# hanmekim/SceneLib2

Hardware: AMD Instinct MI355X
Metric: batched MonoSLAM frames/sec (320x240, 100 feat) (higher is better)
Workload: dtype f64

## Files before the change

### include/scenelib2_amd_testing.h

```cpp
#ifndef SCENELIB2_AMD_TESTING_H
#define SCENELIB2_AMD_TESTING_H
#include "scenelib2_amd.h"
#ifdef __cplusplus
extern "C" {
#endif

int sl2_set_feature_counters(sl2_engine* e, int seq, int label, int attempted, int successful);

int sl2_debug_set_position_error(sl2_engine* e, int seq, int label, int err);

int sl2_debug_graph_captures(sl2_engine* e);

int sl2_debug_update_plan(sl2_engine* e, int group, int* out, int n);

int sl2_debug_raw_covariance(sl2_engine* e, int seq, double* P, int capacity_ld, int* ld);

int sl2_debug_ncc_score(int device, const int32_t* sums5, int count, double* score, double* sd0, double* sd1);
int sl2_debug_gemm_kt(int device, const double* XT, int ldx, const double* YT, int ldy, int M, int N, int K,
                      double* C, int ldc);

int sl2_debug_microbench(int device, int which, double* result);

#define SL2_FRAME_MONITOR_BAND_ROWS 32

#ifdef __cplusplus
}
#endif
#endif
```

### scenelib2_amd/_lib.py

```python
import ctypes as C
import os

import numpy as np

_HERE = os.path.dirname(os.path.abspath(__file__))
LIB_PATH = os.environ.get("SL2_LIB_PATH") or os.path.join(_HERE, "libscenelib2_amd.so")

SL2_OK = 0
SL2_ERR_INVALID = 1
SL2_ERR_HIP = 2
SL2_ERR_CAPACITY = 3
SL2_ERR_NO_DEVICE = 4


class Sl2Error(RuntimeError):
    def __init__(self, code, msg):
        super().__init__("scenelib2_amd error %d: %s" % (code, msg))
        self.code = code


class sl2_camera(C.Structure):
    _fields_ = [("width", C.c_int32), ("height", C.c_int32), ("fku", C.c_double), ("fkv", C.c_double),
                ("u0", C.c_double), ("v0", C.c_double), ("kd1", C.c_double), ("sd", C.c_int32)]

# ... 106 lines not shown
                               ("rgb", np.uint8, (3,)), ("pad", np.uint8), ("q", np.float64, (4,))])
assert OVERLAY_ITEM_DTYPE.itemsize == 64
SL2_WORLD_TRAJECTORY, SL2_WORLD_FEATURES, SL2_WORLD_UNCERTAINTIES, SL2_WORLD_CAMERA, SL2_WORLD_AXES, SL2_WORLD_ALL = 1, 2, 4, 8, 16, 31


class sl2_view(C.Structure):
    _fields_ = [("r", C.c_double * 3), ("q", C.c_double * 4), ("fku", C.c_double), ("fkv", C.c_double), ("u0", C.c_double),
                ("v0", C.c_double)]


VIEW_DTYPE = np.dtype([("r", np.float64, (3,)), ("q", np.float64, (4,)), ("fku", np.float64), ("fkv", np.float64),
                       ("u0", np.float64), ("v0", np.float64)])
assert C.sizeof(sl2_view) == 88 and VIEW_DTYPE.itemsize == 88

SL2_BLOB_MAGIC = 0x51324C53
SL2_BLOB_SLOT_ARRAYS = 22
SL2_BLOB_LAYOUT_OFFSETS = 7 + SL2_BLOB_SLOT_ARRAYS

assert C.sizeof(sl2_snapshot_header) == 256 and C.sizeof(sl2_partial_info) == 32 and C.sizeof(sl2_sequence_blob_header) == 256
assert C.sizeof(sl2_step_stats) == 96 and STEP_STATS_DTYPE.itemsize == 96
assert C.sizeof(sl2_frame_source) == 24

EXPORTED_SYMBOLS = [
    "sl2_api_version", "sl2_device_count", "sl2_create", "sl2_destroy", "sl2_last_error", "sl2_synchronize", "sl2_batch",
    "sl2_max_features", "sl2_set_vehicle_state", "sl2_get_vehicle_state", "sl2_add_known_features", "sl2_set_feature_covariances",
    "sl2_go_one_step", "sl2_initialise_feature", "sl2_initialise_auto_feature", "sl2_save_patch", "sl2_set_groups", "sl2_set_search_variant", "sl2_set_step_fusion", "sl2_get_stream", "sl2_set_search_split", "sl2_set_update_variant", "sl2_set_graph_mode", "sl2_kalman_filter_predict", "sl2_auto_select_n_features", "sl2_make_measurements",
    "sl2_kalman_filter_update", "sl2_finish_step", "sl2_elliptical_search_batch", "sl2_find_best_patch_batch",
    "sl2_search_multiple_overlapping_ellipses_batch", "sl2_list_frames", "sl2_read_pgm", "sl2_read_image", "sl2_ingest_open",
    "sl2_ingest_frame_count", "sl2_ingest_next", "sl2_ingest_set_zero_copy", "sl2_ingest_close", "sl2_get_total_state_sizes",
    "sl2_get_total_state", "sl2_get_total_covariance", "sl2_get_features", "sl2_get_partial_feature", "sl2_get_selection",
    "sl2_snapshot_capacity", "sl2_snapshot", "sl2_get_trajectory", "sl2_get_feature_patch", "sl2_get_position_log", "sl2_delete_features", "sl2_get_status_flags", "sl2_set_profiling", "sl2_set_profile_focus",
    "sl2_reset_kernel_times", "sl2_kernel_count", "sl2_get_kernel_time", "sl2_get_step_work", "sl2_get_placement",
    "sl2_synth_render_host", "sl2_synth_render_device", "sl2_dev_malloc", "sl2_dev_free", "sl2_dev_upload",
    "sl2_dev_download",
    "sl2_sequence_blob_layout", "sl2_sequence_blob_capacity", "sl2_save_sequences", "sl2_load_sequences", "sl2_copy_sequences",
    "sl2_reset_sequences",
    "sl2_set_active_sequences", "sl2_get_active_sequences", "sl2_ingest_frame_counts", "sl2_ingest_next_ragged",
    "sl2_get_step_stats",
    "sl2_set_delta_t", "sl2_get_delta_t", "sl2_set_pause_catch_up",
    "sl2_set_cameras", "sl2_get_cameras",
    "sl2_converter_create", "sl2_converter_destroy", "sl2_converter_set_sources", "sl2_converter_get_sources",
    "sl2_convert_frames", "sl2_convert_frame_host", "sl2_scale_camera",
    "sl2_converter_set_filters", "sl2_converter_get_filters", "sl2_convert_frame_host_filtered",
    "sl2_snapshot_bound", "sl2_snapshot_batch",
    "sl2_overlay_item_bound", "sl2_overlay_items", "sl2_draw_items_batch", "sl2_draw_overlays", "sl2_draw_items_host",
    "sl2_rectify_frames", "sl2_rectify_frame_host", "sl2_scene_item_bound", "sl2_scene_items", "sl2_draw_rectified",
    "sl2_view_look_at", "sl2_world_item_bound", "sl2_world_items", "sl2_draw_world", "sl2_pick_items_batch", "sl2_pick_items_host",
    "sl2_converter_set_map", "sl2_converter_set_remaps", "sl2_converter_get_remaps", "sl2_remap_frame_host",
    "sl2_lens_map_host", "sl2_lens_pinhole_camera",
    "sl2_frame_monitor_create", "sl2_frame_monitor_destroy", "sl2_frame_monitor_set_gates", "sl2_frame_monitor_get_gates",
    "sl2_frame_monitor_reset", "sl2_examine_frames", "sl2_frame_monitor_read", "sl2_frame_stats_host", "sl2_frame_verdict_host",
]
TEST_SYMBOLS = ["sl2_set_feature_counters", "sl2_debug_set_position_error", "sl2_debug_ncc_score", "sl2_debug_gemm_kt", "sl2_debug_microbench", "sl2_debug_graph_captures",
                "sl2_debug_update_plan", "sl2_debug_raw_covariance"]
TEST_LIB_PATH = os.path.join(_HERE, "libscenelib2_amd_test.so")
_testlib = None

_lib = None

c_dp = C.POINTER(C.c_double)
c_ip = C.POINTER(C.c_int32)
c_u8p = C.POINTER(C.c_uint8)
vp = C.c_void_p


def dp(a):
    return a.ctypes.data_as(c_dp)


def ip(a):
    return a.ctypes.data_as(c_ip)


def u8p(a):
    return a.ctypes.data_as(c_u8p)


def _bind(L):
    L.sl2_last_error.restype = C.c_char_p
    L.sl2_device_count.restype = C.c_int
    L.sl2_create.argtypes = [C.POINTER(sl2_camera), C.POINTER(sl2_params), C.c_int, C.c_int, C.c_int, vp, C.POINTER(vp)]
    L.sl2_destroy.argtypes = [vp]
    L.sl2_destroy.restype = None
    L.sl2_synchronize.argtypes = [vp]
    L.sl2_batch.argtypes = [vp]
    L.sl2_max_features.argtypes = [vp]
    L.sl2_set_vehicle_state.argtypes = [vp, C.c_int, C.c_int, c_dp, c_dp]
    L.sl2_get_vehicle_state.argtypes = [vp, C.c_int, C.c_int, c_dp, c_dp]
    L.sl2_add_known_features.argtypes = [vp, C.c_int, C.c_int, C.c_int, c_dp, c_dp, c_u8p]
    L.sl2_set_feature_covariances.argtypes = [vp, C.c_int, C.c_int, C.c_int, c_dp]
    L.sl2_go_one_step.argtypes = [vp, vp, C.c_size_t, C.c_int, C.c_int, C.c_int]
    L.sl2_set_groups.argtypes = [vp, C.c_int]
    L.sl2_set_search_variant.argtypes = [vp, C.c_int]
    if "SL2_LIB_PATH" not in os.environ or hasattr(L, "sl2_set_search_split"):
        L.sl2_set_search_split.argtypes = [vp, C.c_int]
    L.sl2_set_update_variant.argtypes = [vp, C.c_int, C.c_int]
    L.sl2_set_graph_mode.argtypes = [vp, C.c_int]
    L.sl2_set_step_fusion.argtypes = [vp, C.c_int]
    L.sl2_get_stream.argtypes = [vp]
    L.sl2_get_stream.restype = vp
    L.sl2_kalman_filter_predict.argtypes = [vp]
    L.sl2_auto_select_n_features.argtypes = [vp, C.c_int]
    L.sl2_make_measurements.argtypes = [vp, vp, C.c_size_t, C.c_int]
    L.sl2_kalman_filter_update.argtypes = [vp]
    L.sl2_finish_step.argtypes = [vp, C.c_int]
    L.sl2_elliptical_search_batch.argtypes = [C.c_int, c_u8p, C.c_int, C.c_int, C.c_int, c_ip, c_u8p, c_dp, c_dp,
                                              C.c_int, c_ip, c_ip, c_dp, C.c_int]
# ... 92 lines not shown
        L.sl2_overlay_item_bound.argtypes = [C.c_int, C.c_int]
        L.sl2_overlay_item_bound.restype = C.c_size_t
        L.sl2_overlay_items.argtypes = [vp, C.c_int, C.c_int, C.c_int, vp, vp, C.c_int, vp, C.c_int]
        L.sl2_draw_items_batch.argtypes = [C.c_int, vp, vp, C.c_int, C.c_int, C.c_int, C.c_int, C.c_size_t, vp, C.c_int, vp, C.c_int,
                                           vp, C.c_size_t, C.c_int, vp, C.c_size_t, C.c_int]
        L.sl2_draw_overlays.argtypes = [vp, C.c_int, C.c_int, vp, C.c_size_t, C.c_int, C.c_int, vp, vp, C.c_size_t, C.c_int]
        L.sl2_draw_items_host.argtypes = [vp, C.c_int, C.c_int, vp, C.c_int, vp, C.c_size_t, C.c_int, vp]
    if "SL2_LIB_PATH" not in os.environ or hasattr(L, "sl2_rectify_frames"):
        L.sl2_rectify_frames.argtypes = [vp, C.c_int, C.c_int, vp, C.c_size_t, C.c_int, vp, C.c_size_t, C.c_int]
        L.sl2_rectify_frame_host.argtypes = [vp, C.c_int, C.c_int, C.c_double, C.c_double, C.c_double, vp]
        L.sl2_scene_item_bound.argtypes = [C.c_int, C.c_int]
        L.sl2_scene_item_bound.restype = C.c_size_t
        L.sl2_scene_items.argtypes = [vp, C.c_int, C.c_int, C.c_int, vp, vp, C.c_int, vp, C.c_int]
        L.sl2_draw_rectified.argtypes = [vp, C.c_int, C.c_int, vp, C.c_size_t, C.c_int, C.c_int, vp, vp, C.c_size_t, C.c_int]
    if "SL2_LIB_PATH" not in os.environ or hasattr(L, "sl2_world_items"):
        L.sl2_view_look_at.argtypes = [c_dp, c_dp, c_dp, C.c_double, C.c_double, C.c_double, C.c_double, vp]
        L.sl2_world_item_bound.argtypes = [C.c_int, C.c_int]
        L.sl2_world_item_bound.restype = C.c_size_t
        L.sl2_world_items.argtypes = [vp, C.c_int, C.c_int, vp, C.c_int, C.c_int, vp, vp, C.c_int, vp, vp, C.c_int]
        L.sl2_draw_world.argtypes = [vp, C.c_int, C.c_int, vp, C.c_int, C.c_int, C.c_int, C.c_int, C.c_int, vp, vp, C.c_size_t, C.c_int]
        L.sl2_pick_items_batch.argtypes = [C.c_int, vp, C.c_int, C.c_int, C.c_int, vp, C.c_int, vp, C.c_int, vp, vp, C.c_int]
        L.sl2_pick_items_host.argtypes = [C.c_int, C.c_int, vp, C.c_int, C.c_int, C.c_int, C.c_int, vp]
    if "SL2_LIB_PATH" not in os.environ or hasattr(L, "sl2_examine_frames"):
        L.sl2_frame_monitor_create.argtypes = [C.c_int, C.c_int, C.c_int, C.c_int, C.POINTER(vp)]
        L.sl2_frame_monitor_destroy.argtypes = [vp]
        L.sl2_frame_monitor_destroy.restype = None
        L.sl2_frame_monitor_set_gates.argtypes = [vp, C.c_int, C.c_int, C.POINTER(sl2_frame_gate)]
        L.sl2_frame_monitor_get_gates.argtypes = [vp, C.c_int, C.c_int, C.POINTER(sl2_frame_gate)]
        L.sl2_frame_monitor_reset.argtypes = [vp, C.c_int, C.c_int]
        L.sl2_examine_frames.argtypes = [vp, vp, vp, C.c_size_t, vp, vp, vp, vp]
        L.sl2_frame_monitor_read.argtypes = [vp, C.c_int, C.c_int, vp, vp]
        L.sl2_frame_stats_host.argtypes = [vp, C.c_int, C.c_int, C.POINTER(sl2_frame_stats)]
        L.sl2_frame_verdict_host.argtypes = [C.POINTER(sl2_frame_stats), C.POINTER(sl2_frame_gate), C.c_int, C.c_uint64]
        L.sl2_frame_verdict_host.restype = C.c_uint32
    return L


def load_testing():
    global _testlib
    if _testlib is not None:
        return _testlib
    load()
    if not os.path.exists(TEST_LIB_PATH):
        raise ImportError("scenelib2_amd: %s not built (make -C scenelib2_amd/csrc)" % TEST_LIB_PATH)
    T = _bind(C.CDLL(TEST_LIB_PATH))
    T.sl2_set_feature_counters.argtypes = [vp, C.c_int, C.c_int, C.c_int, C.c_int]
    T.sl2_debug_set_position_error.argtypes = [vp, C.c_int, C.c_int, C.c_int]
    T.sl2_debug_ncc_score.argtypes = [C.c_int, c_ip, C.c_int, c_dp, c_dp, c_dp]
    T.sl2_debug_gemm_kt.argtypes = [C.c_int, c_dp, C.c_int, c_dp, C.c_int, C.c_int, C.c_int, C.c_int, c_dp, C.c_int]
    T.sl2_debug_microbench.argtypes = [C.c_int, C.c_int, c_dp]
    T.sl2_debug_graph_captures.argtypes = [vp]
    T.sl2_debug_update_plan.argtypes = [vp, C.c_int, c_ip, C.c_int]
    T.sl2_debug_raw_covariance.argtypes = [vp, C.c_int, c_dp, C.c_int, c_ip]
    _testlib = T
    return T


def load():
    global _lib
    if _lib is not None:
        return _lib
    if not os.path.exists(LIB_PATH):
        raise ImportError("scenelib2_amd: native library %s not built (run __graft_entry__.build() or "
                          "`make -C scenelib2_amd/csrc`); there is no CPU fallback" % LIB_PATH)
    _lib = _bind(C.CDLL(LIB_PATH))
    return _lib


def check(rc, L=None):
    if rc != SL2_OK:
        raise Sl2Error(rc, (L or load()).sl2_last_error().decode("utf-8", "replace"))


def device_count():
    return load().sl2_device_count()


def make_camera(cam):
    return sl2_camera(int(cam["width"]), int(cam["height"]), float(cam["fku"]), float(cam["fkv"]),
                      float(cam["u0"]), float(cam["v0"]), float(cam["kd1"]), int(cam["sd"]))


def make_params(p):
    d = dict(delta_t=0.0, number_of_features_to_select=10, number_of_features_to_keep_visible=12,
             max_features_to_init_at_once=1, min_lambda=0.5, max_lambda=5.0, number_of_particles=100,
             standard_deviation_depth_ratio=0.3, min_number_of_particles=20, prune_probability_threshold=0.05,
             erase_partially_init_feature_after_this_many_attempts=10,
             minimum_attempted_measurements_of_feature=10, successful_match_fraction=0.5)
    d.update({k: v for k, v in p.items() if k in d})
    return sl2_params(float(d["delta_t"]), int(d["number_of_features_to_select"]),
                      int(d["number_of_features_to_keep_visible"]), int(d["max_features_to_init_at_once"]),
                      float(d["min_lambda"]), float(d["max_lambda"]), int(d["number_of_particles"]),
                      float(d["standard_deviation_depth_ratio"]), int(d["min_number_of_particles"]),
                      float(d["prune_probability_threshold"]),
                      int(d["erase_partially_init_feature_after_this_many_attempts"]),
                      int(d["minimum_attempted_measurements_of_feature"]), float(d["successful_match_fraction"]))


class DeviceBuffer:

    def __init__(self, nbytes, device=0):
        self.device = device
        self.nbytes = int(nbytes)
        p = vp()
        check(load().sl2_dev_malloc(device, self.nbytes, C.byref(p)))
        self.ptr = p.value
# ... 23 lines not shown
```

### scenelib2_amd/csrc/sl2_common.hpp

```cpp
#pragma once
#include <hip/hip_runtime.h>

#include <cstdio>
#include <cstring>
#include <string>
#include <vector>

#include "../../include/scenelib2_amd.h"
#include "sl2_math.hpp"
#include "sl2_seq_arrays.hpp"
#include "sl2_step_plan.hpp"
#include "sl2_update_plan.hpp"

namespace sl2 {

void set_error(const std::string& s);
const char* hip_err_text(hipError_t e);

#define SL2_HIP(call)                                                                          \
  do {                                                                                         \
    hipError_t _e = (call);                                                                    \
    if (_e != hipSuccess) {                                                                    \
      char _buf[512];                                                                          \
      snprintf(_buf, sizeof(_buf), "%s:%d: %s -> %s", __FILE__, __LINE__, #call, hipGetErrorString(_e)); \
// ... 60 lines not shown
  return cam;
}
#endif

struct KernelTimer {
  std::string name;
  double total_ms = 0.0;
  int64_t launches = 0;
};
struct PendingEvent {
  int timer;
  hipEvent_t start, stop;
};

}

struct sl2_engine : sl2::SeqArrays {
  int device = 0;
  hipStream_t stream = nullptr;
  bool own_stream = false;
  sl2::CameraParams cam;
  sl2_params prm;
  int B = 0;
  int N = 0;
  int ld = 0;
  int nsel_max = 0;
  int mld = 0;
  int nblk_max = 0;
  long long steps_done = 0;
  int chol_variant = 1;
  void* chol_trace = nullptr;
  int build_variant = 1;
  int fwd_variant = 1;
  int ppos = 0;
  int kpart = 1;
  int pcap = 128;
  double* score_map = nullptr;
  int* me_big_list = nullptr;
  int* me_big_count = nullptr;
  bool mapping_used = false;
  int* init_uv = nullptr;
  struct StepGraph { const void* frames; size_t stride; sl2::StepPlan plan; hipGraphExec_t exec; };
  bool graph_mode = false;
  std::vector<StepGraph> step_graphs;
  long long graph_captures = 0;
  int build_split = 0;
  int score_threads = 0;
  int no_ksplit = 0;
  int panel_from = 16;
  int group_from = sl2::kFwdLdsMaxBlocks;
  int fwd_group = 8;
  int chol_panel = 8;
  int build_ahead = 1;
  int build_lds_min = 0;
  int search_lds_pad = 0;
  int search_chunk = 0;
  int search_variant = 1;
  int* slots_max_dev = nullptr;
  unsigned long long* slots_mail = nullptr;
  unsigned long long* slots_mail_dev = nullptr;
  unsigned long long* parts_mail = nullptr;
  unsigned long long* parts_mail_dev = nullptr;
  int place_candidates = 0;
  float place_syrk_ms[2] = {0, 0};
  float place_kept_ms[4] = {0, 0, 0, 0};
  float place_worst_ms[3] = {0, 0, 0};
  long long parts_block_step = -1;
  int slots_exact = 0;
  long long slots_exact_step = 0;
  int step_fusion = 1;
  int search_split = sl2::kSrchSplitDefault;
  int* srch_big = nullptr;
  std::vector<sl2_camera> cams_host;
  void* stats_host = nullptr;
  void* stats_host_dev = nullptr;

  void* snap_stage = nullptr;
  void* snap_host = nullptr;
  void* snap_host_dev = nullptr;
  size_t snap_cap = 0;
  unsigned long long snap_ticket = 0;
  void* snapb_stage = nullptr;
  size_t snapb_stage_bytes = 0;
  void* snapb_aux = nullptr;
  void* snapb_aux_host = nullptr;
  void* ovl_lists = nullptr;
  size_t ovl_lists_bytes = 0;
  void* ovl_images = nullptr;
  size_t ovl_images_bytes = 0;
  void* acc_dev = nullptr;
  size_t acc_dev_bytes = 0;
  void* acc_host = nullptr;
  size_t acc_host_bytes = 0;
  void* ckpt_stage = nullptr;
  size_t ckpt_stage_bytes = 0;
  hipEvent_t ckpt_event = nullptr;

  uint8_t* frames_buf = nullptr;
  const uint8_t* cur_frames = nullptr;
  size_t cur_stride = 0;

  bool profiling = false;
  int profile_level = 2;
  std::string profile_focus;
  std::vector<sl2::KernelTimer> timers;
  std::vector<sl2::PendingEvent> pending;
  std::vector<hipEvent_t> event_pool;

  sl2_engine* root = nullptr;
  std::vector<sl2_engine*> groups;
  int group_first = 0;
  hipEvent_t fork_event = nullptr;

  int timer_id(const char* name);
  void prof_begin(int id, hipStream_t st);
  void prof_end(hipStream_t st);
  int fold_events();
  int sync_all();
};

namespace sl2 {

inline const SeqArrays& seq_arrays(const sl2_engine* e) { return *e; }

struct LaunchScope {
  sl2_engine* e;
  bool on;
  size_t slot = 0;
  static bool wanted(const sl2_engine* r, const char* name, bool major) {
    if (!r->profiling) return false;
    if (r->profile_level >= 2) return true;
    if (!major) return false;
    if (r->profile_focus.empty()) return true;
    return r->profile_focus.find(std::string(",") + name + ",") != std::string::npos;
  }
  LaunchScope(sl2_engine* eng, const char* name, bool major = false) : e(eng), on(wanted(eng->root, name, major)) {
    if (on) { e->root->prof_begin(e->root->timer_id(name), e->stream); slot = e->root->pending.size() - 1; }
  }
  ~LaunchScope() {
    if (on) hipEventRecord(e->root->pending[slot].stop, e->stream);
  }
};

int launch_predict(sl2_engine* e);
int launch_feature_prediction(sl2_engine* e);
int launch_select(sl2_engine* e, int n);
int launch_search(sl2_engine* e);
int launch_search_kernel(sl2_engine* e);
int launch_search_score(sl2_engine* e);
int launch_small_front(sl2_engine* e, int n);
int launch_small_back(sl2_engine* e, int save_trajectory, int panel_w);
int launch_update(sl2_engine* e);
constexpr int kNoProductForm = -1;
int launch_build(sl2_engine* e, const UpdatePlan& p);
int launch_factor(sl2_engine* e, const UpdatePlan& p);
int launch_substitute(sl2_engine* e, const UpdatePlan& p);
int launch_product(sl2_engine* e);
int launch_panel_solve(sl2_engine* e, int pb, int p0, int c0, int ntile, int nb);
int launch_syrk_on(sl2_engine* e, const double* Vt, double* P);
UpdateShape update_shape(const sl2_engine* e);
int launch_build_two_pass(sl2_engine* e, int threads);
int launch_chol_per_block(sl2_engine* e);
int launch_fwdsub_reread(sl2_engine* e);
int launch_finalize(sl2_engine* e, int save_trajectory);
int launch_mapping(sl2_engine* e, const TailPlan& tp);
int launch_manual_init(sl2_engine* e, const int* d_uv);
int launch_auto_init(sl2_engine* e);
int launch_compact_slots(sl2_engine* e, int need, bool honour_mask = false);
int checkpoint_refresh_slots(sl2_engine* e);
int checkpoint_drop_graphs(sl2_engine* e);
int checkpoint_enable_mapping(sl2_engine* e);
void release_checkpoint_staging(sl2_engine* e);
int write_grey_image(const char* path, const uint8_t* px, int w, int h);

}
```

### scenelib2_amd/csrc/sl2_engine.hip

```cpp
#include "sl2_common.hpp"
#include "sl2_mapmath.hpp"

#include <mutex>

namespace sl2 {

static thread_local std::string g_err;
void set_error(const std::string& s) { g_err = s; }


__global__ void k_add_features(double* __restrict__ x, double* __restrict__ xp_org, uint8_t* __restrict__ patch,
                               int* __restrict__ patch_sums, int* __restrict__ f_flags, int* __restrict__ n_slots,
                               int* __restrict__ attempted, int* __restrict__ successful, int* __restrict__ f_label,
                               int* __restrict__ next_label, const double* __restrict__ y_in,
                               const double* __restrict__ xp_in, const uint8_t* __restrict__ patch_in, int seq0, int nfeat,
                               int N, int ld) {
  const int s = blockIdx.x, b = seq0 + s;
  const int base = n_slots[b];
  const int base_label = next_label[b];
  for (int f = threadIdx.x; f < nfeat; f += blockDim.x) {
    const int slot = base + f;
    const size_t fi = (size_t)b * N + slot;
    const size_t src = (size_t)s * nfeat + f;
    for (int k = 0; k < 3; ++k) x[(size_t)b * ld + 13 + 3 * slot + k] = y_in[src * 3 + k];
// ... 1265 lines not shown
  return write_grey_image(path, patch, SL2_PATCH_SIZE, SL2_PATCH_SIZE);
}

int sl2_get_trajectory(sl2_engine* e, int seq, double* out, int capacity, int* count) {
  if (!range_ok(e, seq, 1) || !out || !count) return SL2_ERR_INVALID;
  SL2_HIP(hipSetDevice(e->device));
  { int _rc = e->sync_all(); if (_rc != SL2_OK) return _rc; }
  int total = 0;
  SL2_HIP(hipMemcpy(&total, e->traj_count + seq, sizeof(int), hipMemcpyDeviceToHost));
  std::vector<double> ring((size_t)kTrajCapacity * 3);
  SL2_HIP(hipMemcpy(ring.data(), e->traj + (size_t)seq * kTrajCapacity * 3, sizeof(double) * ring.size(), hipMemcpyDeviceToHost));
  int have = total < kTrajCapacity ? total : kTrajCapacity;
  int n = have < capacity ? have : capacity;
  for (int i = 0; i < n; ++i) {
    const int logical = total - n + i;
    const int slot = logical % kTrajCapacity;
    for (int k = 0; k < 3; ++k) out[i * 3 + k] = ring[(size_t)slot * 3 + k];
  }
  *count = n;
  return SL2_OK;
}

int sl2_get_position_log(sl2_engine* e, int seq0, int nseq, double* out, int capacity, int* count) {
  if (!range_ok(e, seq0, nseq) || !out || !count || capacity <= 0) return SL2_ERR_INVALID;
  SL2_HIP(hipSetDevice(e->device));
  { int _rc = e->sync_all(); if (_rc != SL2_OK) return _rc; }
  const long long total = e->steps_done;
  const int have = (int)(total < kTrajCapacity ? total : kTrajCapacity);
  const int n = have < capacity ? have : capacity;
  std::vector<double> ring((size_t)nseq * kTrajCapacity * 3);
  SL2_HIP(hipMemcpy(ring.data(), e->pos_log + (size_t)seq0 * kTrajCapacity * 3, sizeof(double) * ring.size(), hipMemcpyDeviceToHost));
  for (int s = 0; s < nseq; ++s)
    for (int i = 0; i < n; ++i) {
      const int slot = (int)((total - n + i) % kTrajCapacity);
      for (int k = 0; k < 3; ++k) out[((size_t)s * n + i) * 3 + k] = ring[((size_t)s * kTrajCapacity + slot) * 3 + k];
    }
  *count = n;
  return SL2_OK;
}

#ifdef SL2_TESTING
int sl2_debug_graph_captures(sl2_engine* e) { return e ? (int)e->graph_captures : -1; }

int sl2_debug_raw_covariance(sl2_engine* e, int seq, double* P, int capacity_ld, int* ld) {
  if (!range_ok(e, seq, 1) || !P || !ld) return SL2_ERR_INVALID;
  *ld = e->ld;
  if (e->ld > capacity_ld) return SL2_ERR_CAPACITY;
  SL2_HIP(hipSetDevice(e->device));
  { int _rc = e->sync_all(); if (_rc != SL2_OK) return _rc; }
  SL2_HIP(hipMemcpy(P, e->P + (size_t)seq * e->ld * e->ld, sizeof(double) * e->ld * e->ld, hipMemcpyDeviceToHost));
  return SL2_OK;
}

int sl2_set_feature_counters(sl2_engine* e, int seq, int label, int attempted, int successful) {
  if (!range_ok(e, seq, 1) || label < 0) return SL2_ERR_INVALID;
  SL2_HIP(hipSetDevice(e->device));
  int slot = -1;
  { int _rc = slot_of_label(e, seq, label, &slot); if (_rc != SL2_OK) return _rc; }
  if (slot < 0) return SL2_ERR_INVALID;
  SL2_HIP(hipMemcpy(e->attempted + (size_t)seq * e->N + slot, &attempted, sizeof(int), hipMemcpyHostToDevice));
  SL2_HIP(hipMemcpy(e->successful + (size_t)seq * e->N + slot, &successful, sizeof(int), hipMemcpyHostToDevice));
  return SL2_OK;
}
int sl2_debug_set_position_error(sl2_engine* e, int seq, int label, int err) {
  if (!range_ok(e, seq, 1) || label < 0 || err < 0 || err % 3) return SL2_ERR_INVALID;
  SL2_HIP(hipSetDevice(e->device));
  int slot = -1;
  { int _rc = slot_of_label(e, seq, label, &slot); if (_rc != SL2_OK) return _rc; }
  if (slot < 0) return SL2_ERR_INVALID;
  const int one = 1;
  SL2_HIP(hipMemcpy(e->pos_err + (size_t)seq * e->N + slot, &err, sizeof(int), hipMemcpyHostToDevice));
  if (err) SL2_HIP(hipMemcpy(e->pos_err_any + seq, &one, sizeof(int), hipMemcpyHostToDevice));
  return SL2_OK;
}
#endif

__global__ void __launch_bounds__(256) k_delete_feature(double* __restrict__ P, int* __restrict__ f_flags, const int* __restrict__ f_label,
                                                        const int* __restrict__ n_slots, const int* __restrict__ labels,
                                                        int* __restrict__ done, int N, int ld) {
  const int b = blockIdx.x;
  const int lab = labels[b];
  __shared__ int s_slot;
  if (threadIdx.x == 0) s_slot = -1;
  __syncthreads();
  if (lab >= 0)
    for (int f = threadIdx.x; f < n_slots[b]; f += blockDim.x) {
      const int fl = f_flags[(size_t)b * N + f];
      if ((fl & FF_ACTIVE) && !(fl & FF_PARTIAL) && f_label[(size_t)b * N + f] == lab) s_slot = f;
    }
  __syncthreads();
  const int slot = s_slot;
  const bool ok = slot >= 0;
  if (threadIdx.x == 0) { done[b] = ok ? 1 : 0; if (ok) f_flags[(size_t)b * N + slot] = FF_USED; }
  if (!ok) return;
  double* Pb = P + (size_t)b * ld * ld;
  const int pos = 13 + 3 * slot;
  for (int j = threadIdx.x; j < ld; j += blockDim.x)
    for (int r = 0; r < 3; ++r) {
      Pb[(size_t)(pos + r) * ld + j] = 0.0;
      Pb[(size_t)j * ld + pos + r] = 0.0;
    }
}

int sl2_delete_features(sl2_engine* e, int seq0, int nseq, const int32_t* labels, int32_t* deleted) {
  if (!range_ok(e, seq0, nseq) || !labels) return SL2_ERR_INVALID;
  SL2_HIP(hipSetDevice(e->device));
// ... 169 lines not shown
```

### scenelib2_amd/csrc/sl2_update_syrk.hip

```cpp
#include "sl2_update_dev.hpp"

namespace sl2 {


__global__ void __launch_bounds__(256, 4) k_syrk(const double* __restrict__ Vt, double* __restrict__ P, double* __restrict__ x,
                                              const int* __restrict__ m_count, int ld, int mld, int B,
                                              const int* __restrict__ n_slots, int ppos
#ifdef SL2_CHOL_TRACE
                                              , long long* trace
#endif
                                              ) {
#ifdef SL2_CHOL_TRACE
  struct Stamp {
    long long* p;
    __device__ Stamp(long long* q) : p(q) { if (p && threadIdx.x == 0) p[2 * blockIdx.x] = (long long)__builtin_readcyclecounter(); }
    __device__ ~Stamp() { if (p && threadIdx.x == 0) p[2 * blockIdx.x + 1] = (long long)__builtin_readcyclecounter(); }
  } stamp(trace);
#endif
  int b, t;
  const int ntl = ld / 64;
  if (!xcd_map(ntl * (ntl + 1) / 2, B, &b, &t)) return;
  const int cnt = m_count[b];
  if (cnt == 0) return;
  const int mp = (2 * cnt + kSyrkKC - 1) / kSyrkKC * kSyrkKC;
  const int nks_last = (2 * cnt - (mp - kSyrkKC) + 3) >> 2;
  int tj = 0;
  while (t > tj) { t -= tj + 1; ++tj; }
  const int ti = t;
  const int n_live = 13 + 3 * n_slots[b];
  {
    const int t_lo = (n_live + 63) >> 6, t_hi = ppos >> 6;
    if ((ti >= t_lo && ti < t_hi) || (tj >= t_lo && tj < t_hi)) return;
  }
  const int tid = threadIdx.x;
  const int lane = tid & 63, wave = tid >> 6;
  const int lo = lane & 15, hi = lane >> 4;
  const int wi = (wave >> 1) * 32, wj = (wave & 1) * 32;
  const double* Vb = Vt + (size_t)b * mld * ld;
  double* Pb = P + (size_t)b * ld * ld;
  __shared__ double sAB[2][2][kSyrkKC * 64];
  const int kr = tid >> 4, c2 = (tid & 15) * 2;
  const double* gA = Vb + (size_t)kr * ld + ti * 64 + c2;
  const double* gB = Vb + (size_t)kr * ld + tj * 64 + c2;
  struct Stage { double2 a0, a1, b0, b1; };
  auto stage_load = [&](int chunk) {
    Stage r;
    const size_t off = (size_t)chunk * kSyrkKC * ld;
    r.a0 = *(const double2*)(gA + off); r.a1 = *(const double2*)(gA + off + 32);
    r.b0 = *(const double2*)(gB + off); r.b1 = *(const double2*)(gB + off + 32);
    return r;
  };
  auto stage_store = [&](int buf, const Stage& r) {
    const int cs = c2 ^ ((kr & 1) << 4);
// ... 65 lines not shown
        if (!plain(it, jt)) continue;
#pragma unroll
        for (int r = 0; r < 4; ++r) {
          if (diagw && it == 1 && jt == 0) continue;
          const double pn = pold[it][jt][r] - acc[it][jt][r];
          prow[(size_t)(16 * it + 4 * r) * ld + 16 * jt] = pn;
          acc[it][jt][r] = pn;
        }
      }
    if (mirror || diagw) {
      const int other = lastbuf ^ 1;
      double* sM = &sAB[other][0][0] + wave * (16 * 17);
      double* pm = Pb + (size_t)(j0 + hi) * ld + i0 + lo;
#pragma unroll
      for (int it = 0; it < 2; ++it)
#pragma unroll
        for (int jt = 0; jt < 2; ++jt) {
          if (diagw && !(it == 0 && jt == 1)) continue;
          if (!plain(it, jt)) continue;
#pragma unroll
          for (int r = 0; r < 4; ++r) sM[lo * 17 + 4 * r + hi] = acc[it][jt][r];
          asm volatile("s_waitcnt lgkmcnt(0)" ::: "memory");
#pragma unroll
          for (int k = 0; k < 4; ++k) pm[(size_t)(16 * jt + 4 * k) * ld + 16 * it] = sM[(4 * k + hi) * 17 + lo];
          asm volatile("s_waitcnt lgkmcnt(0)" ::: "memory");
        }
    }
    if (interior) return;
  }
  double* xb = x + (size_t)b * ld;
#pragma unroll
  for (int it = 0; it < 2; ++it)
#pragma unroll
    for (int jt = 0; jt < 2; ++jt) {
      if (plain(it, jt)) continue;
#pragma unroll
      for (int r = 0; r < 4; ++r) {
        const int row = i0 + 16 * it + hi + 4 * r, col = j0 + 16 * jt + lo;
        const double v = acc[it][jt][r];
        if (col == ld - 1) {
          if (row != ld - 1) xb[row] += v;
        } else if (row != ld - 1) {
          const double pn = pold[it][jt][r] - v;
          Pb[(size_t)row * ld + col] = pn;
          if (mirror) Pb[(size_t)col * ld + row] = pn;
        }
      }
    }
}

int launch_product(sl2_engine* e) {
  const int B = e->B;
  LaunchScope ls(e, "k_syrk", true);
  const int nt = e->ld / 64;
#ifdef SL2_CHOL_TRACE
  static const bool trace_syrk = getenv("SL2_TRACE_SYRK") != nullptr;
  hipLaunchKernelGGL(k_syrk, dim3(xcd_grid(nt * (nt + 1) / 2, B)), dim3(256), 0, e->stream, e->Vt, e->P, e->x, e->m_gate,
                     e->ld, e->mld, B, e->n_slots, e->ppos, trace_syrk ? (long long*)e->root->chol_trace : nullptr);
#else
  hipLaunchKernelGGL(k_syrk, dim3(xcd_grid(nt * (nt + 1) / 2, B)), dim3(256), 0, e->stream, e->Vt, e->P, e->x, e->m_gate,
                     e->ld, e->mld, B, e->n_slots, e->ppos);
#endif
  SL2_HIP(hipGetLastError());
  return SL2_OK;
}

int launch_syrk_on(sl2_engine* e, const double* Vt, double* P) {
  const int nt = e->ld / 64;
#ifdef SL2_CHOL_TRACE
  hipLaunchKernelGGL(k_syrk, dim3(xcd_grid(nt * (nt + 1) / 2, e->B)), dim3(256), 0, e->stream, Vt, P, e->x, e->m_count, e->ld, e->mld, e->B,
                     e->n_slots, e->ppos, (long long*)nullptr);
#else
  hipLaunchKernelGGL(k_syrk, dim3(xcd_grid(nt * (nt + 1) / 2, e->B)), dim3(256), 0, e->stream, Vt, P, e->x, e->m_count, e->ld, e->mld, e->B,
                     e->n_slots, e->ppos);
#endif
  SL2_HIP(hipGetLastError());
  return SL2_OK;
}

}
```

### scenelib2_amd/monoslam.py

```python
import ctypes as C

import os

import numpy as np

from . import _lib
from .config import load_config, read_pgm, resolve_identifier


def decode_snapshot(raw):
    h = _lib.sl2_snapshot_header.from_buffer_copy(raw[:256])
    assert h.magic == 0x53324C53 and 256 <= h.bytes <= len(raw)
    has = lambda bit: not (h.omitted_sections & bit)
    f64 = lambda off, n: np.frombuffer(raw, dtype=np.float64, count=n, offset=off).copy()
    out = dict(header=h, xv=f64(h.off_xv, 13), Pxx=f64(h.off_Pxx, 169).reshape(13, 13), features=[], partial=[], patches={})
    fsz = C.sizeof(_lib.sl2_feature_info)
    cov = h.off_cov
    for i in range(h.n_features if has(_lib.SL2_SNAP_FEATURES) else 0):
        f = _lib.sl2_feature_info.from_buffer_copy(raw[h.off_features + i * fsz: h.off_features + (i + 1) * fsz])
        d = f.state_size
        Pxy = Pyy = None
        if has(_lib.SL2_SNAP_COV):
            Pxy = f64(cov, 13 * d).reshape(13, d)
            Pyy = f64(cov + 13 * d * 8, d * d).reshape(d, d)
# ... 415 lines not shown

    def selection(self, seq):
        labels = np.zeros(self.max_features, dtype=np.int32)
        counters = np.zeros(3, dtype=np.int32)
        self._ck(self.L.sl2_get_selection(self.h, seq, _lib.ip(labels), self.max_features, _lib.ip(counters)))
        return labels[:counters[1]].copy(), dict(visible=int(counters[0]), selected=int(counters[1]),
                                                 measurement_size=int(counters[2]))

    def trajectory(self, seq, capacity=1000):
        out = np.zeros((capacity, 3))
        cnt = C.c_int(0)
        self._ck(self.L.sl2_get_trajectory(self.h, seq, _lib.dp(out), capacity, C.byref(cnt)))
        return out[:cnt.value].copy()

    def position_log(self, seq0=0, nseq=None, capacity=1000):
        nseq = self.batch - seq0 if nseq is None else nseq
        out = np.zeros((nseq, capacity, 3))
        cnt = C.c_int(0)
        self._ck(self.L.sl2_get_position_log(self.h, seq0, nseq, _lib.dp(out), capacity, C.byref(cnt)))
        return out.reshape(-1)[: nseq * cnt.value * 3].reshape(nseq, cnt.value, 3).copy()

    def set_feature_counters(self, seq, label, attempted, successful):
        T = _lib.load_testing()
        _lib.check(T.sl2_set_feature_counters(self.h, seq, label, attempted, successful), T)

    def debug_set_position_error(self, seq, label, err):
        T = _lib.load_testing()
        _lib.check(T.sl2_debug_set_position_error(self.h, seq, label, err), T)

    UPDATE_PLAN_FIELDS = ("build", "build_threads", "build_nsplit", "build_lds_bytes", "chol", "chol_panel_blocks",
                          "fwd", "fwd_nb", "fwd_group_rows")
    BUILD_FORMS = ("two-pass", "<1,4>", "<2,2>", "ahead<4>", "ahead<2>")
    CHOL_FORMS = ("none", "left", "panels", "per-block")
    FWD_FORMS = ("none", "ksplit", "lds", "grouped", "re-read")

    def debug_update_plan(self, group=0):
        T = _lib.load_testing()
        out = np.zeros(len(self.UPDATE_PLAN_FIELDS), dtype=np.int32)
        _lib.check(T.sl2_debug_update_plan(self.h, group, _lib.ip(out), out.size), T)
        p = dict(zip(self.UPDATE_PLAN_FIELDS, (int(v) for v in out)))
        p.update(build=self.BUILD_FORMS[p["build"]], chol=self.CHOL_FORMS[p["chol"]], fwd=self.FWD_FORMS[p["fwd"]])
        return p

    def debug_raw_covariance(self, seq):
        T = _lib.load_testing()
        ld = np.zeros(1, dtype=np.int32)
        P = np.zeros((1, 1))
        if T.sl2_debug_raw_covariance(self.h, seq, _lib.dp(P), 1, _lib.ip(ld)) != _lib.SL2_ERR_CAPACITY:
            raise RuntimeError("sl2_debug_raw_covariance: no size reported")
        P = np.zeros((int(ld[0]), int(ld[0])))
        _lib.check(T.sl2_debug_raw_covariance(self.h, seq, _lib.dp(P), P.shape[0], _lib.ip(ld)), T)
        return P

    def delete_features(self, labels, seq0=0):
        lab = np.ascontiguousarray(labels, dtype=np.int32)
        done = np.zeros(lab.size, dtype=np.int32)
        self._ck(self.L.sl2_delete_features(self.h, int(seq0), lab.size, _lib.ip(lab), _lib.ip(done)))
        return done.astype(bool)

    def initialise_feature(self, frames, uv, on_device=False, seq_stride=0):
        ptr, stride, dev, keep = self._frames_arg(frames, seq_stride, on_device)
        sel = np.ascontiguousarray(uv, dtype=np.int32).reshape(self.batch, 2)
        created = np.zeros(self.batch, dtype=np.int32)
        self._ck(self.L.sl2_initialise_feature(self.h, ptr, stride, dev, _lib.ip(sel), _lib.ip(created)))
        return created.astype(bool)

    def initialise_auto_feature(self, frames, on_device=False, seq_stride=0):
        ptr, stride, dev, keep = self._frames_arg(frames, seq_stride, on_device)
        created = np.zeros(self.batch, dtype=np.int32)
        self._ck(self.L.sl2_initialise_auto_feature(self.h, ptr, stride, dev, _lib.ip(created)))
        return created.astype(bool)

    def save_patch(self, seq, label, path):
        self._ck(self.L.sl2_save_patch(self.h, int(seq), int(label), os.fsencode(path)))

    def feature_patch(self, seq, label):
        out = np.zeros((11, 11), dtype=np.uint8)
        self._ck(self.L.sl2_get_feature_patch(self.h, int(seq), int(label), _lib.u8p(out)))
        return out

    def status_flags(self):
        out = np.zeros(self.batch, dtype=np.int32)
        self._ck(self.L.sl2_get_status_flags(self.h, 0, self.batch, _lib.ip(out)))
        return out

    def step_stats(self, seq0=0, nseq=None):
        nseq = self.batch - seq0 if nseq is None else int(nseq)
        out = np.zeros(max(nseq, 1), dtype=_lib.STEP_STATS_DTYPE)
        self._ck(self.L.sl2_get_step_stats(self.h, int(seq0), nseq, out.ctypes.data_as(_lib.vp), 0))
        return out[:nseq]

    def step_stats_device(self, dev_ptr, seq0=0, nseq=None):
        nseq = self.batch - seq0 if nseq is None else int(nseq)
        self._ck(self.L.sl2_get_step_stats(self.h, int(seq0), nseq, _lib.vp(int(dev_ptr)), 1))

    def sequence_blob_capacity(self):
        return int(self.L.sl2_sequence_blob_capacity(self.h))

    def save_sequences(self, seq0=0, nseq=None):
        nseq = self.batch - seq0 if nseq is None else int(nseq)
        cap = self.sequence_blob_capacity()
        buf = np.zeros((max(nseq, 1), cap), dtype=np.uint8)
        sizes = np.zeros(max(nseq, 1), dtype=np.uint64)
        self._ck(self.L.sl2_save_sequences(self.h, int(seq0), nseq, buf.ctypes.data_as(_lib.vp), cap, 0,
                                           sizes.ctypes.data_as(C.POINTER(C.c_uint64))))
        return [buf[i, :int(sizes[i])].tobytes() for i in range(nseq)]
# ... 394 lines not shown
```

Measured before the change: 1.048 million.

## Add strip-based SYRK kernel pairing adjacent tiles per workgroup for covariance update

```diff
diff --git a/include/scenelib2_amd_testing.h b/include/scenelib2_amd_testing.h
--- a/include/scenelib2_amd_testing.h
+++ b/include/scenelib2_amd_testing.h
@@ -15,6 +15,8 @@
 
 int sl2_debug_raw_covariance(sl2_engine* e, int seq, double* P, int capacity_ld, int* ld);
 
+int sl2_debug_set_syrk_form(sl2_engine* e, int form);
+
 int sl2_debug_ncc_score(int device, const int32_t* sums5, int count, double* score, double* sd0, double* sd1);
 int sl2_debug_gemm_kt(int device, const double* XT, int ldx, const double* YT, int ldy, int M, int N, int K,
                       double* C, int ldc);
diff --git a/scenelib2_amd/_lib.py b/scenelib2_amd/_lib.py
--- a/scenelib2_amd/_lib.py
+++ b/scenelib2_amd/_lib.py
@@ -182,7 +182,7 @@
     "sl2_frame_monitor_reset", "sl2_examine_frames", "sl2_frame_monitor_read", "sl2_frame_stats_host", "sl2_frame_verdict_host",
 ]
 TEST_SYMBOLS = ["sl2_set_feature_counters", "sl2_debug_set_position_error", "sl2_debug_ncc_score", "sl2_debug_gemm_kt", "sl2_debug_microbench", "sl2_debug_graph_captures",
-                "sl2_debug_update_plan", "sl2_debug_raw_covariance"]
+                "sl2_debug_update_plan", "sl2_debug_raw_covariance", "sl2_debug_set_syrk_form"]
 TEST_LIB_PATH = os.path.join(_HERE, "libscenelib2_amd_test.so")
 _testlib = None
 
@@ -381,6 +381,7 @@
     T.sl2_debug_graph_captures.argtypes = [vp]
     T.sl2_debug_update_plan.argtypes = [vp, C.c_int, c_ip, C.c_int]
     T.sl2_debug_raw_covariance.argtypes = [vp, C.c_int, c_dp, C.c_int, c_ip]
+    T.sl2_debug_set_syrk_form.argtypes = [vp, C.c_int]
     _testlib = T
     return T
 
diff --git a/scenelib2_amd/csrc/sl2_common.hpp b/scenelib2_amd/csrc/sl2_common.hpp
--- a/scenelib2_amd/csrc/sl2_common.hpp
+++ b/scenelib2_amd/csrc/sl2_common.hpp
@@ -136,6 +136,7 @@
   int fwd_group = 8;
   int chol_panel = 8;
   int build_ahead = 1;
+  int syrk_form = -1;
   int build_lds_min = 0;
   int search_lds_pad = 0;
   int search_chunk = 0;
@@ -240,6 +241,7 @@
 int launch_factor(sl2_engine* e, const UpdatePlan& p);
 int launch_substitute(sl2_engine* e, const UpdatePlan& p);
 int launch_product(sl2_engine* e);
+int launch_product_strip(sl2_engine* e);
 int launch_panel_solve(sl2_engine* e, int pb, int p0, int c0, int ntile, int nb);
 int launch_syrk_on(sl2_engine* e, const double* Vt, double* P);
 UpdateShape update_shape(const sl2_engine* e);
diff --git a/scenelib2_amd/csrc/sl2_engine.hip b/scenelib2_amd/csrc/sl2_engine.hip
--- a/scenelib2_amd/csrc/sl2_engine.hip
+++ b/scenelib2_amd/csrc/sl2_engine.hip
@@ -1341,6 +1341,15 @@
   return SL2_OK;
 }
 
+int sl2_debug_set_syrk_form(sl2_engine* e, int form) {
+  if (!e || form < -1 || form > 1) return SL2_ERR_INVALID;
+  e = e->root;
+  SL2_HIP(hipSetDevice(e->device));
+  { int rc = drop_step_graphs(e); if (rc != SL2_OK) return rc; }
+  e->syrk_form = form;
+  return SL2_OK;
+}
+
 int sl2_set_feature_counters(sl2_engine* e, int seq, int label, int attempted, int successful) {
   if (!range_ok(e, seq, 1) || label < 0) return SL2_ERR_INVALID;
   SL2_HIP(hipSetDevice(e->device));
diff --git a/scenelib2_amd/csrc/sl2_syrk_strip_plan.hpp b/scenelib2_amd/csrc/sl2_syrk_strip_plan.hpp
--- /dev/null
+++ b/scenelib2_amd/csrc/sl2_syrk_strip_plan.hpp
@@ -0,0 +1,57 @@
+#pragma once
+
+#if defined(__HIPCC__)
+#define SL2_STRIP_HD __host__ __device__
+#else
+#define SL2_STRIP_HD
+#endif
+
+namespace sl2 {
+
+constexpr int kStripKC = 16;
+constexpr int kStripMinWorkgroups = 768;
+
+struct StripPass { int ti, tj, width; };
+
+SL2_STRIP_HD inline int strip_row_passes(int nt, int ti) { return (nt - ti + 1) / 2; }
+
+SL2_STRIP_HD inline int strip_pass_count(int nt) {
+  int n = 0;
+  for (int ti = 0; ti < nt; ++ti) n += strip_row_passes(nt, ti);
+  return n;
+}
+
+SL2_STRIP_HD inline StripPass strip_pass(int nt, int pass) {
+  int ti = 0;
+  while (ti < nt && pass >= strip_row_passes(nt, ti)) { pass -= strip_row_passes(nt, ti); ++ti; }
+  StripPass p = {ti, ti, 0};
+  if (ti >= nt) return p;
+  const int off = nt - ti - 1;
+  if (off & 1) {
+    p.tj = ti + 2 * pass; p.width = 2;
+  } else if (pass == 0) {
+    p.width = 1;
+  } else {
+    p.tj = ti + 1 + 2 * (pass - 1); p.width = 2;
+  }
+  return p;
+}
+
+SL2_STRIP_HD inline bool syrk_tile_dead(int ti, int tj, int t_lo, int t_hi) {
+  return (ti >= t_lo && ti < t_hi) || (tj >= t_lo && tj < t_hi);
+}
+
+SL2_STRIP_HD inline StripPass strip_trim(StripPass p, int t_lo, int t_hi) {
+  if (p.width == 2 && syrk_tile_dead(p.ti, p.tj + 1, t_lo, t_hi)) p.width = 1;
+  if (p.width >= 1 && syrk_tile_dead(p.ti, p.tj, t_lo, t_hi)) { p.tj += 1; p.width -= 1; }
+  return p;
+}
+
+inline bool syrk_takes_strip(int ld, int group_B, int forced) {
+  const int nt = ld / 64;
+  if (forced >= 0) return forced != 0;
+  if (nt < 2) return false;
+  return (long long)strip_pass_count(nt) * group_B >= kStripMinWorkgroups;
+}
+
+}
diff --git a/scenelib2_amd/csrc/sl2_update_syrk.hip b/scenelib2_amd/csrc/sl2_update_syrk.hip
--- a/scenelib2_amd/csrc/sl2_update_syrk.hip
+++ b/scenelib2_amd/csrc/sl2_update_syrk.hip
@@ -1,4 +1,5 @@
 #include "sl2_update_dev.hpp"
+#include "sl2_syrk_strip_plan.hpp"
 
 namespace sl2 {
 
@@ -170,6 +171,7 @@
 int launch_product(sl2_engine* e) {
   const int B = e->B;
   LaunchScope ls(e, "k_syrk", true);
+  if (syrk_takes_strip(e->ld, B, e->root->syrk_form)) return launch_product_strip(e);
   const int nt = e->ld / 64;
 #ifdef SL2_CHOL_TRACE
   static const bool trace_syrk = getenv("SL2_TRACE_SYRK") != nullptr;
diff --git a/scenelib2_amd/csrc/sl2_update_syrk_strip.hip b/scenelib2_amd/csrc/sl2_update_syrk_strip.hip
--- /dev/null
+++ b/scenelib2_amd/csrc/sl2_update_syrk_strip.hip
@@ -0,0 +1,205 @@
+#include "sl2_update_dev.hpp"
+#include "sl2_syrk_strip_plan.hpp"
+
+namespace sl2 {
+
+template <int KC>
+__global__ void __launch_bounds__(256, KC == 16 ? 3 : 4)
+k_syrk_strip(const double* __restrict__ Vt, double* __restrict__ P, double* __restrict__ x, const int* __restrict__ m_count,
+             int ld, int mld, int B, const int* __restrict__ n_slots, int ppos) {
+  static_assert(KC == 8 || KC == 16, "two k-steps or four per chunk");
+  constexpr int TPR = 256 / KC;
+  constexpr int kBuf = KC * 192;
+  int b, t;
+  const int ntl = ld / 64;
+  if (!xcd_map(strip_pass_count(ntl), B, &b, &t)) return;
+  const int cnt = m_count[b];
+  if (cnt == 0) return;
+  const int mp = (2 * cnt + KC - 1) / KC * KC;
+  const int nks_last = (2 * cnt - (mp - KC) + 3) >> 2;
+  const int n_live = 13 + 3 * n_slots[b];
+  const StripPass pass = strip_trim(strip_pass(ntl, t), (n_live + 63) >> 6, ppos >> 6);
+  if (pass.width == 0) return;
+  const int ti = pass.ti, tj = pass.tj;
+  const bool wide = pass.width == 2;
+  const int tid = threadIdx.x;
+  const int lane = tid & 63, wave = __builtin_amdgcn_readfirstlane(tid >> 6);
+  const int lo = lane & 15, hi = lane >> 4;
+  const int wi = (wave >> 1) * 32, wj = (wave & 1) * (wide ? 64 : 32);
+  const double* Vb = Vt + (size_t)b * mld * ld;
+  double* Pb = P + (size_t)b * ld * ld;
+  __shared__ double sAB[2][kBuf];
+  const int kr = tid / TPR, c2 = (tid % TPR) * 2;
+  const double* gA = Vb + (size_t)kr * ld + ti * 64 + c2;
+  const double* gB = Vb + (size_t)kr * ld + tj * 64 + c2;
+  struct Stage { double2 a0, a1, b0, b1, b2, b3; };
+  auto ldg = [](const double* p) { return *(const double2*)p; };
+  const double2 zero2 = make_double2(0.0, 0.0);
+  auto stage_load = [&](int chunk) {
+    Stage r;
+    const double* pA = gA + (size_t)chunk * KC * ld;
+    const double* pB = gB + (size_t)chunk * KC * ld;
+    if constexpr (KC == 16) {
+      r.a0 = ldg(pA); r.a1 = ldg(pA + 32);
+      r.b0 = ldg(pB); r.b1 = ldg(pB + 32);
+      r.b2 = wide ? ldg(pB + 64) : zero2; r.b3 = wide ? ldg(pB + 96) : zero2;
+    } else {
+      r.a0 = ldg(pA); r.a1 = zero2;
+      r.b0 = ldg(pB); r.b1 = wide ? ldg(pB + 64) : zero2;
+      r.b2 = zero2; r.b3 = zero2;
+    }
+    return r;
+  };
+  auto stage_store = [&](int buf, const Stage& r) {
+    const int cs = c2 ^ ((kr & 1) << 4);
+    double* dA = &sAB[buf][kr * 64 + cs];
+    double* dB = &sAB[buf][KC * 64 + kr * 128 + cs];
+    if constexpr (KC == 16) {
+      *(double2*)dA = r.a0; *(double2*)(dA + 32) = r.a1;
+      *(double2*)dB = r.b0; *(double2*)(dB + 32) = r.b1; *(double2*)(dB + 64) = r.b2; *(double2*)(dB + 96) = r.b3;
+    } else {
+      *(double2*)dA = r.a0;
+      *(double2*)dB = r.b0; *(double2*)(dB + 64) = r.b1;
+    }
+  };
+  Stage r0 = stage_load(0);
+  const int i0 = ti * 64 + wi;
+  const int b_lo = (n_live + 31) >> 5, b_hi = ppos >> 5;
+  int jc[2];
+  bool live[2], diagw[2], interior[2];
+#pragma unroll
+  for (int jb = 0; jb < 2; ++jb) {
+    jc[jb] = tj * 64 + wj + 32 * jb;
+    live[jb] = (jb == 0 || wide) && jc[jb] >= i0 && !((i0 >> 5) >= b_lo && (i0 >> 5) < b_hi) &&
+               !((jc[jb] >> 5) >= b_lo && (jc[jb] >> 5) < b_hi);
+    interior[jb] = (i0 + 32 < ld && jc[jb] + 32 < ld);
+    diagw[jb] = (jc[jb] == i0) && interior[jb];
+  }
+  const bool idle = !live[0] && !live[1];
+  v4d acc[2][4];
+#pragma unroll
+  for (int it = 0; it < 2; ++it)
+#pragma unroll
+    for (int jq = 0; jq < 4; ++jq) acc[it][jq] = (v4d){0, 0, 0, 0};
+  const int nchunk = mp / KC;
+  Stage r1 = r0;
+  if (nchunk > 1) r1 = stage_load(1);
+  auto chunk_mfma = [&](int buf, int nks) {
+    const int sw = (hi & 1) << 4;
+    const double* pa = &sAB[buf][hi * 64 + wi + lo];
+    const double* pb = &sAB[buf][KC * 64 + hi * 128 + wj + lo];
+#pragma unroll
+    for (int ks = 0; ks < KC / 4; ++ks) {
+      if (ks < nks) {
+        const double a0 = pa[ks * 256 + sw], a1 = pa[ks * 256 + (sw ^ 16)];
+#pragma unroll
+        for (int jb = 0; jb < 2; ++jb) {
+          if (!live[jb]) continue;
+          const double b0 = pb[ks * 512 + 32 * jb + sw], b1 = pb[ks * 512 + 32 * jb + (sw ^ 16)];
+          acc[0][2 * jb] = mfma_f64(a0, b0, acc[0][2 * jb]);
+          acc[0][2 * jb + 1] = mfma_f64(a0, b1, acc[0][2 * jb + 1]);
+          if (!diagw[jb]) acc[1][2 * jb] = mfma_f64(a1, b0, acc[1][2 * jb]);
+          acc[1][2 * jb + 1] = mfma_f64(a1, b1, acc[1][2 * jb + 1]);
+        }
+      }
+    }
+  };
+  for (int ch = 0; ch < nchunk; ch += 2) {
+    stage_store(0, r0);
+    __syncthreads();
+    if (ch + 2 < nchunk) r0 = stage_load(ch + 2);
+    if (!idle) chunk_mfma(0, (ch + 1 >= nchunk) ? nks_last : KC / 4);
+    if (ch + 1 >= nchunk) break;
+    stage_store(1, r1);
+    __syncthreads();
+    if (ch + 3 < nchunk) r1 = stage_load(ch + 3);
+    if (!idle) chunk_mfma(1, (ch + 2 >= nchunk) ? nks_last : KC / 4);
+  }
+  if (idle) return;
+  const int lastbuf = (nchunk - 1) & 1;
+  constexpr bool kFetchBoth = KC == 16;
+  double pold[kFetchBoth ? 2 : 1][2][2][4];
+  auto Pat = [&](unsigned row, unsigned col) -> double& { return *(double*)((char*)Pb + ((row * (unsigned)ld + col) << 3)); };
+  auto fetch_block = [&](int jb) {
+#pragma unroll
+    for (int it = 0; it < 2; ++it)
+#pragma unroll
+      for (int jt = 0; jt < 2; ++jt)
+#pragma unroll
+        for (int r = 0; r < 4; ++r) pold[kFetchBoth ? jb : 0][it][jt][r] = Pat(i0 + hi + 16 * it + 4 * r, jc[jb] + lo + 16 * jt);
+  };
+  if (kFetchBoth) {
+#pragma unroll
+    for (int jb = 0; jb < 2; ++jb)
+      if (live[jb]) fetch_block(jb);
+  }
+  double* sM = &sAB[lastbuf ^ 1][0] + wave * (16 * 17);
+  double* xb = x + (size_t)b * ld;
+#pragma unroll
+  for (int jb = 0; jb < 2; ++jb) {
+    if (!live[jb]) continue;
+    if (!kFetchBoth) fetch_block(jb);
+    const int pb = kFetchBoth ? jb : 0;
+    const int j0 = jc[jb];
+    const bool inter = interior[jb], dg = diagw[jb];
+    const bool mirror = j0 != i0;
+    auto plain = [&](int it, int jt) { return inter || ((i0 + 16 * it + 16 < ld) && (j0 + 16 * jt + 16 < ld)); };
+#pragma unroll
+    for (int it = 0; it < 2; ++it)
+#pragma unroll
+      for (int jt = 0; jt < 2; ++jt) {
+        if (!plain(it, jt)) continue;
+#pragma unroll
+        for (int r = 0; r < 4; ++r) {
+          if (dg && it == 1 && jt == 0) continue;
+          const double pn = pold[pb][it][jt][r] - acc[it][2 * jb + jt][r];
+          Pat(i0 + hi + 16 * it + 4 * r, j0 + lo + 16 * jt) = pn;
+          acc[it][2 * jb + jt][r] = pn;
+        }
+      }
+    if (mirror || dg) {
+#pragma unroll
+      for (int it = 0; it < 2; ++it)
+#pragma unroll
+        for (int jt = 0; jt < 2; ++jt) {
+          if (dg && !(it == 0 && jt == 1)) continue;
+          if (!plain(it, jt)) continue;
+#pragma unroll
+          for (int r = 0; r < 4; ++r) sM[lo * 17 + 4 * r + hi] = acc[it][2 * jb + jt][r];
+          asm volatile("s_waitcnt lgkmcnt(0)" ::: "memory");
+#pragma unroll
+          for (int k = 0; k < 4; ++k) Pat(j0 + hi + 16 * jt + 4 * k, i0 + lo + 16 * it) = sM[(4 * k + hi) * 17 + lo];
+          asm volatile("s_waitcnt lgkmcnt(0)" ::: "memory");
+        }
+    }
+    if (inter) continue;
+#pragma unroll
+    for (int it = 0; it < 2; ++it)
+#pragma unroll
+      for (int jt = 0; jt < 2; ++jt) {
+        if (plain(it, jt)) continue;
+#pragma unroll
+        for (int r = 0; r < 4; ++r) {
+          const int row = i0 + 16 * it + hi + 4 * r, col = j0 + 16 * jt + lo;
+          const double v = acc[it][2 * jb + jt][r];
+          if (col == ld - 1) {
+            if (row != ld - 1) xb[row] += v;
+          } else if (row != ld - 1) {
+            const double pn = pold[pb][it][jt][r] - v;
+            Pat(row, col) = pn;
+            if (mirror) Pat(col, row) = pn;
+          }
+        }
+      }
+  }
+}
+
+int launch_product_strip(sl2_engine* e) {
+  const int np = strip_pass_count(e->ld / 64);
+  hipLaunchKernelGGL(k_syrk_strip<kStripKC>, dim3(xcd_grid(np, e->B)), dim3(256), 0, e->stream, e->Vt, e->P, e->x, e->m_gate, e->ld,
+                     e->mld, e->B, e->n_slots, e->ppos);
+  SL2_HIP(hipGetLastError());
+  return SL2_OK;
+}
+
+}
diff --git a/scenelib2_amd/monoslam.py b/scenelib2_amd/monoslam.py
--- a/scenelib2_amd/monoslam.py
+++ b/scenelib2_amd/monoslam.py
@@ -491,6 +491,10 @@
         _lib.check(T.sl2_debug_raw_covariance(self.h, seq, _lib.dp(P), P.shape[0], _lib.ip(ld)), T)
         return P
 
+    def debug_set_syrk_form(self, form):
+        T = _lib.load_testing()
+        _lib.check(T.sl2_debug_set_syrk_form(self.h, int(form)), T)
+
     def delete_features(self, labels, seq0=0):
         lab = np.ascontiguousarray(labels, dtype=np.int32)
         done = np.zeros(lab.size, dtype=np.int32)
```

Result: slower. 1.027 million (-2.0%).
